# aharmat/mcptam

Measured on AMD Instinct MI355X. Metric: ChainBundle LM iters/sec (4-cam, 200 MKF, 50k pts, 400k meas) @1/2/4/8 GPU, higher is better.
Workload: dtype f64; 1 GPU; metric: 4 cams, 200 MKF, 50000 points, 400000 measurements per rank; parallelism=points sharded x1, poses replicated, allreduce_transport=none

## Files before the change

### include/mcp_ba.h

```cpp
#ifndef MCP_BA_H
#define MCP_BA_H

#include <stddef.h>

#ifdef __cplusplus
extern "C" {
#endif

#define MCP_MAX_CHAIN 8
#define MCP_MAX_INV   31

typedef struct mcp_camera {
  double params[9];
  double image_size[2];
  double affine[4];
  double center[2];
  double min_theta;
  double max_rho;
  double theta_mean;
  double theta_std;
  int    n_inv;
  int    pad_;
  double inv_coeffs[MCP_MAX_INV];
} mcp_camera;
// ... 92 lines not shown
void mcp_ba_struct_cache_stats(long long* hits, long long* misses);
long long mcp_ba_struct_cache_near_hits(void);
void mcp_ba_struct_cache_clear(void);
int mcp_chol_debug_factor(const double* A, int n, const double* b, double* L_out, double* y_out, int* info);
int mcp_chol_time(const double* A, int n, const double* b, int nsys, int reps, int band, double* ms_factor, double* ms_back, double* x);
int mcp_debug_pose_cut(const unsigned char* adjacency, int nf, int max_arcs, int threads, int* order_out, int* segs_out, int* info_out);
int mcp_ba_debug_system(mcp_ba*, double lambda, double* S_rhs_b_out);
int mcp_ba_debug_systems(mcp_ba*, int nsys, const double* lambdas, double* out);
#define MCP_BA_LIN_NONE  0
#define MCP_BA_LIN_QUAD  1
#define MCP_BA_LIN_PIPE  2
#define MCP_BA_LIN_GROUP 3
#define MCP_BA_SCHUR_NONE  0
#define MCP_BA_SCHUR_4     1
#define MCP_BA_SCHUR_GROUP 2
typedef struct mcp_ba_structure {
  int ngroup, grp_pts, nbig, nfl, np;
  int grp_points_max, grp_points_min;
  int grp_poses_max;
  int grp_no_pose;
  int grp_blk_max, grp_inc_max;
  int lin_kernel;
  int lin_generic;
  int schur_kernel;
  int asm_long;
  int max_systems;
} mcp_ba_structure;
int mcp_ba_debug_structure(mcp_ba*, mcp_ba_structure* out);

#define MCP_BA_HEAD_PLAIN 0
#define MCP_BA_HEAD_RANKS 1
#define MCP_BA_HEAD_RIDE  2
#define MCP_BA_HEAD_SMALL 3
#define MCP_BA_HEAD_AHEAD 4
#define MCP_BA_HEAD_LARGE 5
typedef struct mcp_ba_head_report {
  unsigned long long rank;
  double median;
  double sigma[4];
  double robust_chi2;
  double robust_chi2_plain;
// ... 28 lines not shown
```

### mcptam_amd/chain_bundle.py

```python
import ctypes
import os
import time

import numpy as np

from .taylor_camera import camera_array

_HERE = os.path.dirname(os.path.abspath(__file__))
LIB_PATH = os.environ.get("MCP_HIP_LIB") or os.path.join(_HERE, "libmcptam_hip.so")
_LIB = None

c_double_p = ctypes.POINTER(ctypes.c_double)
c_int_p = ctypes.POINTER(ctypes.c_int)
c_ubyte_p = ctypes.POINTER(ctypes.c_ubyte)


class McpBaParams(ctypes.Structure):
    _fields_ = [("max_iterations", ctypes.c_int), ("max_trials_after_failure", ctypes.c_int),
                ("update_percent_limit", ctypes.c_double), ("update_rms_limit", ctypes.c_double),
                ("min_mestimator_sigma", ctypes.c_double), ("disable_convergence", ctypes.c_int),
                ("device", ctypes.c_int), ("profile", ctypes.c_int)]


class McpBaIterLog(ctypes.Structure):
# ... 6 lines not shown
    _fields_ = [("total_ms", ctypes.c_double), ("structure_ms", ctypes.c_double), ("eval_ms", ctypes.c_double),
                ("select_ms", ctypes.c_double), ("linearize_ms", ctypes.c_double), ("schur_ms", ctypes.c_double),
                ("cholesky_ms", ctypes.c_double), ("solve_ms", ctypes.c_double), ("update_ms", ctypes.c_double),
                ("n_linearize", ctypes.c_int), ("n_trials", ctypes.c_int), ("n_solves", ctypes.c_int),
                ("n_spec_hits", ctypes.c_int),
                ("n_collectives_main", ctypes.c_int), ("n_collectives_spec", ctypes.c_int),
                ("collective_bytes_main", ctypes.c_double), ("collective_bytes_spec", ctypes.c_double),
                ("n_median_fast", ctypes.c_int), ("n_persist_fallbacks", ctypes.c_int),
                ("schur_mfma_per_system", ctypes.c_double), ("schur_flops_structural", ctypes.c_double),
                ("chol_flops_plan", ctypes.c_double), ("chol_chains", ctypes.c_int)]


class McpBaStructure(ctypes.Structure):
    _fields_ = [(f, ctypes.c_int) for f in (
        "ngroup", "grp_pts", "nbig", "nfl", "np", "grp_points_max", "grp_points_min", "grp_poses_max", "grp_no_pose",
        "grp_blk_max", "grp_inc_max", "lin_kernel", "lin_generic", "schur_kernel", "asm_long", "max_systems")]


class McpBaHeadReport(ctypes.Structure):
    _fields_ = [("rank", ctypes.c_ulonglong), ("median", ctypes.c_double), ("sigma", ctypes.c_double * 4),
                ("robust_chi2", ctypes.c_double), ("robust_chi2_plain", ctypes.c_double), ("route_sigma", ctypes.c_double * 4),
                ("head_status", ctypes.c_int), ("overflow", ctypes.c_int), ("pred_ok", ctypes.c_int),
                ("select_overflow", ctypes.c_int), ("n_median_fast", ctypes.c_int), ("declined", ctypes.c_int)]


class McpBaTrialReport(ctypes.Structure):
    _fields_ = [(f, ctypes.c_double) for f in ("robust_chi2", "scale_pose", "scale_point", "scale", "ss_pose", "ss_point", "ss")] + \
               [(f, ctypes.c_int) for f in ("ncb", "nbb", "nchain", "npose", "npoint", "nfl", "np", "nmeas", "small_mode", "given_step")]


HEAD_ROUTES = ("plain", "ranks", "ride", "small", "ahead", "large")
LIN_KERNEL_NAMES = ("none", "quad", "pipe", "group")
SCHUR_KERNEL_NAMES = ("none", "schur4", "schur_group")

ALLREDUCE_FN = ctypes.CFUNCTYPE(ctypes.c_int, ctypes.c_void_p, ctypes.c_void_p, ctypes.c_size_t, ctypes.c_void_p)

BA_SYMBOLS = [
    "mcp_last_error", "mcp_device_count", "mcp_ba_create", "mcp_ba_destroy", "mcp_ba_add_pose", "mcp_ba_add_point",
    "mcp_ba_add_meas", "mcp_ba_add_points", "mcp_ba_add_measurements", "mcp_ba_compute", "mcp_ba_converged",
    "mcp_ba_total_iterations", "mcp_ba_get_point", "mcp_ba_get_pose", "mcp_ba_get_points", "mcp_ba_get_poses",
    "mcp_ba_num_outliers", "mcp_ba_get_outliers", "mcp_ba_sigma_squared", "mcp_ba_mean_chi_squared", "mcp_ba_max_cov",
    "mcp_ba_lambda", "mcp_ba_num_iter_logs", "mcp_ba_get_iter_logs", "mcp_ba_get_timing", "mcp_ba_set_allreduce",
    "mcp_ba_prepare", "mcp_ba_eval", "mcp_ba_robust_chi2", "mcp_ba_debug_solve", "mcp_dense_spd_solve",
    "mcp_dense_spd_stress", "mcp_ba_debug_system", "mcp_ba_debug_systems", "mcp_ba_debug_structure", "mcp_ba_debug_head", "mcp_ba_debug_trial", "mcp_chol_debug_factor", "mcp_chol_time", "mcp_debug_pose_cut",
    "mcp_ba_struct_cache_stats", "mcp_ba_struct_cache_near_hits", "mcp_ba_struct_cache_clear",
    "mcp_comm_unique_id", "mcp_comm_init", "mcp_comm_destroy", "mcp_ba_set_comm", "mcp_comm_allreduce", "mcp_comm_allreduce_lane",
]

# ... 274 lines not shown
        out = np.zeros(max(len(lams), 1) * per)
        if self._L.mcp_ba_debug_systems(self._h, len(lams), _dp(lams), _dp(out)) < 0:
            raise RuntimeError("mcp_ba_debug_systems: " + last_error())
        return [(out[q * per:q * per + n * n].reshape(n, n).copy(), out[q * per + n * n:q * per + n * n + n].copy(),
                 out[q * per + n * n + n:(q + 1) * per].copy()) for q in range(len(lams))]

    def DebugStructure(self):
        st = McpBaStructure()
        if self._L.mcp_ba_debug_structure(self._h, ctypes.byref(st)) < 0:
            raise RuntimeError("mcp_ba_debug_structure: " + last_error())
        d = {f: int(getattr(st, f)) for f, _ in McpBaStructure._fields_}
        d["lin_kernel"] = LIN_KERNEL_NAMES[d["lin_kernel"]]
        d["schur_kernel"] = SCHUR_KERNEL_NAMES[d["schur_kernel"]]
        d["lin_generic"] = bool(d["lin_generic"])
        d["asm_long"] = bool(d["asm_long"])
        return d

    def DebugHead(self, route, chi2, prev_median):
        chi2 = np.ascontiguousarray(chi2, dtype=np.float64).reshape(-1)
        rep = McpBaHeadReport()
        if self._L.mcp_ba_debug_head(self._h, HEAD_ROUTES.index(route), _dp(chi2), len(chi2), float(prev_median), ctypes.byref(rep)) < 0:
            raise RuntimeError("mcp_ba_debug_head: " + last_error())
        d = {f: getattr(rep, f) for f, _ in McpBaHeadReport._fields_}
        d["sigma"] = np.array(rep.sigma[:], dtype=np.float64)
        d["route_sigma"] = np.array(rep.route_sigma[:], dtype=np.float64)
        return d

    def DebugTrial(self, lam, x=None):
        rep = McpBaTrialReport()
        nx = self.Prepare()
# ... 128 lines not shown
```

### mcptam_amd/csrc/ba_group.h

```cpp
#pragma once
#include "ba_kernels.h"

namespace mcp {

__device__ inline int tri(int r, int c) { return r*(r + 1)/2 + c; }
constexpr int GRP_TRI = GRP_DOF*(GRP_DOF + 1)/2;

template <int NT>
__device__ inline void flush_group_blocks(const double* Sl, const double* bl, int grp, const DevProblem& P,
                                          double* __restrict__ st_blocks, double* __restrict__ st_rhs) {
  const int b0 = P.g_blk0[grp], nb = P.g_blk0[grp + 1] - b0;
  for (int e = threadIdx.x; e < nb*36; e += NT) {
    const int slot = e/36, w = e - 36*slot;
    const int pr = P.blk_pair[b0 + slot], la = pr >> 4, lb = pr & 15;
    const int r = w/6, c = w - 6*r;
    st_blocks[(size_t)P.blk_dst[b0 + slot]*36 + w] = (la == lb && c > r) ? 0.0 : Sl[tri(6*la + r, 6*lb + c)];
  }
  for (int i = threadIdx.x; i < GRP_DOF; i += NT) {
    const int d = P.rhs_dst[grp*GRP_LMAX + i/6];
    if (d >= 0) st_rhs[(size_t)d*6 + i%6] = bl[i];
  }
}

template <int NT>
// ... 740 lines not shown
    __syncthreads();
    if (t >= GRP_DOF && t < 2*GRP_DOF) rl[t - GRP_DOF] += racc;
    __syncthreads();
    flush_group_blocks<256>(Sl, rl, grp, P, stS, str);
  }
  SCH_LAP(7);
  SCH_OUT();
}
struct AsmPlan {
  int nfp;
  int ntiles;
  const int* tiles;
  const int* pair_id;
  const int* pr_start;
  const int* po_start;
};

#ifndef ASM_NT
#define ASM_NT 1024
#endif
__global__ void __launch_bounds__(ASM_NT)
k_assemble(AsmPlan A, int np, const double* __restrict__ stU, const double* __restrict__ stb,
           const double* __restrict__ stS, const double* __restrict__ str,
           const double* __restrict__ Ubig ,
           double* __restrict__ S, SysBatch sb) {
  const int q = blockIdx.y;
  S += q*sb.sstride; stS += q*sb.ststride; str += q*sb.strstride;
  const double lam = sb.lambda_init[q];
  const int packed = A.tiles[blockIdx.x];
  const int ti = packed >> 16, tj = packed & 0xffff;
  const size_t n2 = (size_t)np*np;
  for (int e = threadIdx.x; e < 1024; e += ASM_NT) {
    const int row = 32*ti + (e >> 5), col = 32*tj + (e & 31);
    if (col >= np || row > np) continue;
    if (row == np) {
      const int a = col/6, r = col - 6*a;
      double b = 0.0, sr = 0.0;
// ... 30 lines not shown
        }
        for (; k + 4 <= k1; k += 4, pu += 144, pw += 144) {
          const double u0 = pu[0], u1 = pu[36], u2 = pu[72], u3 = pu[108];
          const double w0 = pw[0], w1 = pw[36], w2 = pw[72], w3 = pw[108];
          u += u0; u += u1; u += u2; u += u3;
          w += w0; w += w1; w += w2; w += w3;
        }
        for (; k < k1; ++k, pu += 36, pw += 36) { u += pu[0]; w += pw[0]; }
      }
      v = u - w;
      if (Ubig) v += Ubig[(size_t)row*np + col];
      if (row == col) v += lam;
    }
    S[(size_t)row*np + col] = v;
  }
}

constexpr int ASML_LPE = 8;
__device__ inline double asml_tree8(double v) {
  v += wave_xor<1>(v); v += wave_xor<2>(v); v += __shfl_xor(v, 4, 64);
  return v;
}
__device__ inline double asml_part(const double* __restrict__ p, int stride, int n, int l8) {
  const int c0 = (n*l8)/ASML_LPE, c1 = (n*(l8 + 1))/ASML_LPE;
  double a = 0.0;
  int k = c0;
  p += (size_t)c0*stride;
  for (; k + 4 <= c1; k += 4, p += 4*(size_t)stride) {
    const double x0 = p[0], x1 = p[stride], x2 = p[2*(size_t)stride], x3 = p[3*(size_t)stride];
    a += x0; a += x1; a += x2; a += x3;
// ... 80 lines not shown
```

### mcptam_amd/csrc/ba_solver.hip

```cpp
#include <hip/hip_runtime.h>
#include <algorithm>
#include <array>
#include <atomic>
#include <memory>
#include <mutex>
#include <sched.h>
#include <thread>
#include <cfloat>
#include <chrono>
#include <cmath>
#include <cstdio>
#include <cstdlib>
#include <cstring>
#include <condition_variable>
#include <functional>
#include <list>
#include <map>
#include <string>
#include <vector>

#include "../../include/mcp_ba.h"
#include "ba_pool.h"
#include "ba_kernels.h"
#include "ba_select.h"
// ... 282 lines not shown
  P.ok = P.main && P.spec;
  if (getenv("MCP_BA_TRACE")) fprintf(stderr, "[mcp_ba streams] device %d: %d side streams overlap with the main stream%s\n", device, got, calibrate ? "" : " (not measured)");
  return P;
}

struct StructKey {
  unsigned long long h0 = 0, h1 = 0; int npose = 0, npoint = 0, nmeas = 0, nchain = 0, dev = 0, flags = 0;
  bool operator==(const StructKey& o) const { return h0 == o.h0 && h1 == o.h1 && npose == o.npose && npoint == o.npoint && nmeas == o.nmeas && nchain == o.nchain && dev == o.dev && flags == o.flags; }
};
struct StructEntry {
  StructKey key;
  std::vector<int> pose_unk, pt_unk, fp_pose, fl_point, perm;
  std::vector<unsigned char> pose_active, pt_active, pat;
  std::vector<int> chol_segs;
  int nfp = 0, nfl = 0, np = 0, nx = 0, nsp = 0, ninc = 0, nslot = 0, ngroup = 0, nbig = 0, grp_pts = 0, grp_blk_max = 0, grp_inc_max = 0, nrhs_rows = 0;
  size_t nstage = 0; bool asm_long = false, sch4_ok = false, sch4_order = false;
  double m_total = 0, nfl_total = 0, schur_mfma = 0, schur_flops = 0;
  std::vector<size_t> counts;
  StructKey base;
  std::vector<int, NoInitAlloc<int>> add_point, add_chain, add_cam;
  char* dblock = nullptr; size_t dbytes = 0, dcap = 0; int ddev = -1;
  size_t host_bytes() const { return (pose_unk.size() + pt_unk.size() + fp_pose.size() + fl_point.size() + perm.size() + add_point.size() + add_chain.size() + add_cam.size())*4 + pose_active.size() + pt_active.size() + pat.size(); }
  ~StructEntry() { if (dblock) DevCache::get().put(dblock, dcap, ddev); }
};
class StructCache {
 public:
  static StructCache& get() { static StructCache* c = new StructCache(); return *c; }
  bool enabled() const { return budget_ > 0; }
  std::shared_ptr<StructEntry> find(const StructKey& k) {
    std::lock_guard<std::mutex> lk(mu_);
    for (auto it = lru_.begin(); it != lru_.end(); ++it) if ((*it)->key == k) { auto e = *it; lru_.erase(it); lru_.push_front(e); ++hits_; return e; }
// ... 87 lines not shown
    DevBuf<double> xp, xl, p0, p1, p2;
    bool pre_run = false, ahead_enq = false; unsigned long long pre_ticket = 0;
    hipEvent_t ev_tr = nullptr;
    hipEvent_t ev_wf = nullptr;
    hipStream_t st_tr = nullptr;
    hipStream_t tr_stream = nullptr;
    hipEvent_t head_ev = nullptr; bool head_enq = false; int head_state = -1; unsigned long long head_ticket = 0;
    DevBuf<double> trial; DevBuf<SelState> trstate;
    int pred_ok = 0, ovf = 0;
  };
  SpecLane lane[MAX_SYS];
  int spec_trials = 2;
  DevBuf<double> d_ubig;
  DevBuf<double> d_red;
  DevBuf<double> d_stU, d_stb, d_stS, d_str, d_udiag;
  DevBuf<int> d_g_blk0, d_asm_tiles, d_pair_id, d_pr_start, d_blk_dst, d_po_start, d_rhs_dst;
  DevBuf<unsigned char> d_blk_pair;
  int grp_blk_max = 0;
  int head_ahead_for = -1;
  bool head_ahead_want = false; int dbg_head_ahead = 0;
  int head_ahead(int w);
  int large_head_ahead = 0;
  struct HeadScratch { unsigned int* hist = nullptr; double* vals = nullptr; double* part = nullptr; double* out = nullptr; double* rs = nullptr; };
  HeadScratch hsc[2*MAX_SYS]; DevBuf<double> d_headbuf;
  hipStream_t st_h = nullptr; bool st_h_own = false;
  unsigned long long head_ticket_ctr = 0;
  int head_par = 0, acc_head_q = -1, dbg_head_miss = 0;
  const double* start_blk = nullptr;
  unsigned int* head_hist(int q) { return hsc[head_par*MAX_SYS + q].hist; }
  int enqueue_head(hipStream_t s, int q, int w, bool side);
  int wait_head(int q);
// ... 17 lines not shown
  int grp_lmax_pol = env_on("MCP_BA_GROUP_LMAX13", true) ? S4_LMAX : GRP_LMAX;
  bool sch4_on = env_on("MCP_BA_SCHUR4", true), sch4_ok = false;
  double schur_mfma = 0, schur_flops = 0;
  std::vector<unsigned char> last_pat;
  std::string launch_err;
  void note_launch(const char* k) { const hipError_t e = hipGetLastError(); if (e != hipSuccess && e != hipErrorNotReady && launch_err.empty()) launch_err = std::string(k) + ": " + hipGetErrorString(e); }
  std::shared_ptr<StructEntry> pending_entry;
  StructKey cache_key, cache_base; bool cache_insert = false;
  int n_masked = 0; int near_miss_on = 1;
  unsigned long long med_rank() const { return (unsigned long long)n_masked + (unsigned long long)(m_total/2); }
  DevBuf<int> d_m_last;
  bool lin_pipe = env_on("MCP_BA_LIN_PIPE", true);
  DevBuf<int> d_g_order, d_sp_unk;
  bool sch4_order = false;
  bool asm_long = false;
  int grp_inc_max = 0;
  size_t nstage = 0;
  int nrhs_rows = 0;
  AsmPlan A;
  DevBuf<double> d_V, d_g, d_W, d_Vinv, d_xl, d_xp_good, d_xl_good, d_err;
  DevBuf<double> d_selvals;
  DevBuf<double> d_seltab;
  int sel_cap = 4096;
  DevBuf<double> d_xp_cand;
  DevBuf<double> d_part0, d_part1, d_part2, d_res, d_sigma, d_hist, d_cov;
  static constexpr int MAX_DIAG_PARTS = 256;
  static int max_diag_parts(int np_, int nfl_) { return std::min(MAX_DIAG_PARTS, (std::max(np_, nfl_) + 1023)/1024); }
  DevBuf<unsigned char> d_headl; bool headl_clean = false; int head_large_on = 0; int hl_grid = 0;
  bool use_head_large() const { return head_large_on && robust && !multi() && !small_mode() && P.nmeas > 0 && hl_grid > 0 && d_headl.p != nullptr; }
  int head_large(int w, int off, double* sig_copy2);
// ... 1359 lines not shown
  B.hold_arena(st);
  HostStruct& H = B.H;
#define CP(x) H.x.assign(x.begin(), x.end())
  CP(m_pt); CP(m_chain); CP(m_sp); CP(slot_start); CP(slot_unk); CP(slot_inc); CP(l_i0); CP(l_i1); CP(l_sp); CP(inc_unk); CP(sp_pt); CP(sp_m); CP(sp_i);
  CP(g_sp0); CP(g_pose); CP(g_blk0); CP(pair_id); CP(pr_start); CP(blk_dst); CP(po_start); CP(rhs_dst); CP(m_cam); CP(slot_first); CP(sp_big); CP(slot_lp);
  CP(inc_lp); CP(inc_mixed); CP(blk_pair); CP(m_mask); CP(m_u); CP(m_v); CP(m_om);
#undef CP
  return finish_prepare(B);
}

struct mcp_ba::BlockLayout {
  struct Item { const void* src; size_t bytes, off; bool direct; };
  std::vector<Item> items; std::vector<size_t> counts;
  size_t total = 0, staged = 0; char* base = nullptr;
  static size_t al(size_t x) { return (x + 255) & ~(size_t)255; }
  std::vector<int> chain_len, chain_pose, pose_unk, pt_chain, pt_unk, sp_unk, g_order; std::vector<unsigned char> pt_fixed;
  std::vector<int, NoInitAlloc<int>> m_last;
};

int mcp_ba::finish_prepare(StructBuild& B) {
  pending_entry.reset();
  const int nmeas = B.hit ? B.hit->key.nmeas : B.nmeas;
  const int nblk = (std::max(nmeas, nfl) + 255)/256 + 1;
  BlockLayout L;
  launch_choices(B);
  if (layout_block(B, L)) return -1;
  if (B.hit ? upload_hit_numbers(B, L) : upload_cold(L)) return -1;
  B.lap("  upload enqueued");
  if (!B.hit && cache_insert && make_cache_entry(B, L)) return -1;
  read_call_knobs();
  if (alloc_work_buffers(nmeas, nblk) || head_scratch(nmeas, nblk) || poison_test_aid() || pinned_mailbox(nblk) || zero_fill() || fill_param_blocks(nmeas)) return -1;
  B.lap("alloc+upload");
  return publish(B);
}

void mcp_ba::launch_choices(StructBuild& B) {
  const StructEntry* hit = B.hit.get(); const HostStruct& H = B.H;
  sch4_ok = ngroup > 0;
  if (hit) sch4_ok = hit->sch4_ok;
  else for (int gi = 0; gi < ngroup && sch4_ok; ++gi) if (H.g_pose[(size_t)gi*GRP_LMAX + S4_LMAX] >= 0) sch4_ok = false;
  schur_mfma = schur_flops = 0;
  if (hit) { schur_mfma = hit->schur_mfma; schur_flops = hit->schur_flops; }
  else if ((prm.profile || cache_insert) && ngroup) schur_work(B);
  if (hit) asm_long = hit->asm_long;
  else {
    const size_t npairs = H.pr_start.empty() ? 0 : H.pr_start.size() - 1;
    asm_long = npairs > 0 && nstage >= 48*npairs;
    if (const char* e = getenv("MCP_BA_ASM_LONG")) asm_long = atoi(e) != 0 && npairs > 0;
  }
}

void mcp_ba::schur_work(StructBuild& B) {
  const HostStruct& H = B.H;
  const int T = finish_threads(B.nmeas);
  std::vector<double> pm(T, 0.0), pf(T, 0.0);
  auto body = [&](int tid) {
    double sm = 0, sf = 0;
    for (int gi = (int)((long)ngroup*tid/T), ge = (int)((long)ngroup*(tid + 1)/T); gi < ge; ++gi) {
      int npl = 0; for (int k = 0; k < GRP_LMAX; ++k) if (H.g_pose[(size_t)gi*GRP_LMAX + k] >= 0) npl = k + 1;
      const int ntile = (6*npl + 15)/16;
      for (int s0 = H.g_sp0[gi]; s0 < H.g_sp0[gi + 1]; s0 += 16) {
        unsigned tm = 0;
        for (int sp = s0; sp < std::min(s0 + 16, H.g_sp0[gi + 1]); ++sp) {
          if (H.sp_big[sp]) continue;
// ... 19 lines not shown
  for (int i = 0; i < npoint; ++i) { L.pt_chain[i] = points[i].chain; L.pt_unk[i] = points[i].unk; L.pt_fixed[i] = (unsigned char)points[i].fixed; }
  L.sp_unk.resize(hit ? 0 : nsp);
  if (!hit) for (int sp = 0; sp < nsp; ++sp) L.sp_unk[sp] = H.sp_big[sp] ? -1 : L.pt_unk[H.sp_pt[sp]];
  sch4_order = hit ? hit->sch4_order : (sch4_on && sch4_ok && ngroup > 512 && env_on("MCP_BA_SCHUR4_ORDER", true));
  if (sch4_order && !hit) {
    std::vector<int> cost(ngroup);
    for (int gi = 0; gi < ngroup; ++gi) {
      int npl = 0; for (int k = 0; k < GRP_LMAX; ++k) if (H.g_pose[(size_t)gi*GRP_LMAX + k] >= 0) npl = k + 1;
      const int nt = (6*npl + 15)/16;
      cost[gi] = nt*(nt + 1)/2*((H.g_sp0[gi + 1] - H.g_sp0[gi] + 15)/16);
    }
    L.g_order.resize(ngroup);
    for (int gi = 0; gi < ngroup; ++gi) L.g_order[gi] = gi;
    std::stable_sort(L.g_order.begin(), L.g_order.end(), [&](int a, int b) { return cost[a] > cost[b]; });
  }
  L.m_last.resize(hit ? 0 : nmeas);
  if (!hit) {
    auto& m_last = L.m_last; const int T = finish_threads(nmeas);
    run_ranges(T, [&](int tid) { for (long j = (long)nmeas*tid/T, e = (long)nmeas*(tid + 1)/T; j < e; ++j) { const int oc = H.m_chain[j]; m_last[j] = oc*MAXC + chains[oc].len - 1; } });
  }
}

int mcp_ba::layout_block(StructBuild& B, BlockLayout& L) {
  const StructEntry* hit = B.hit.get(); const HostStruct& H = B.H;
  small_arrays(B, L);
  L.items.reserve(48); L.counts.reserve(48);
  size_t& total = L.total; auto al = BlockLayout::al;
  size_t nadd = 0;
  auto add = [&](auto& dbuf, const auto& vec, bool pinned) {
    using E = typename std::remove_reference<decltype(vec)>::type::value_type;
// ... 8 lines not shown
    if (!direct) L.staged += al(std::max<size_t>(bytes, 1));
    total += al(std::max<size_t>(bytes, 1));
  };
  add(d_cams, cams, false); add(d_chain_len, L.chain_len, false); add(d_chain_pose, L.chain_pose, false); add(d_pose_unk, L.pose_unk, false);
  add(d_pt_chain, L.pt_chain, false); add(d_pt_unk, L.pt_unk, false); add(d_pt_fixed, L.pt_fixed, false);
  add(d_m_pt, H.m_pt, true); add(d_m_chain, H.m_chain, true); add(d_m_cam, H.m_cam, true); add(d_m_mask, H.m_mask, true);
  add(d_m_u, H.m_u, true); add(d_m_v, H.m_v, true); add(d_m_omega, H.m_om, true); add(d_slot_start, H.slot_start, true);
  add(d_slot_unk, H.slot_unk, true); add(d_slot_inc, H.slot_inc, true); add(d_l_i0, H.l_i0, true); add(d_l_i1, H.l_i1, true);
  add(d_inc_unk, H.inc_unk, true); add(d_fl_point, fl_point, false); add(d_sp_pt, H.sp_pt, true); add(d_sp_m, H.sp_m, true);
  add(d_sp_i, H.sp_i, true); add(d_sp_big, H.sp_big, true); add(d_m_sp, H.m_sp, true); add(d_l_sp, H.l_sp, true);
  add(d_g_sp0, H.g_sp0, true); add(d_g_pose, H.g_pose, true); add(d_slot_lp, H.slot_lp, true); add(d_slot_first, H.slot_first, true);
  add(d_inc_lp, H.inc_lp, true); add(d_inc_mixed, H.inc_mixed, true); add(d_g_blk0, H.g_blk0, true); add(d_blk_pair, H.blk_pair, true);
  add(d_asm_tiles, plan.all_tiles, false); add(d_pair_id, H.pair_id, true); add(d_pr_start, H.pr_start, true); add(d_blk_dst, H.blk_dst, true);
  add(d_po_start, H.po_start, true); add(d_rhs_dst, H.rhs_dst, true);
  add(d_sp_unk, L.sp_unk, false); add(d_g_order, L.g_order, false); add(d_m_last, L.m_last, false);
  if (d_struct.alloc(total)) return -1;
  char* const base = L.base = d_struct.p;
  auto fix = [&](auto& dbuf) { dbuf.p = reinterpret_cast<decltype(dbuf.p)>(base + reinterpret_cast<size_t>(dbuf.p)); };
  fix(d_cams); fix(d_chain_len); fix(d_chain_pose); fix(d_pose_unk); fix(d_pt_chain); fix(d_pt_unk); fix(d_pt_fixed);
  fix(d_m_pt); fix(d_m_chain); fix(d_m_cam); fix(d_m_mask); fix(d_m_u); fix(d_m_v); fix(d_m_omega); fix(d_slot_start);
  fix(d_slot_unk); fix(d_slot_inc); fix(d_l_i0); fix(d_l_i1); fix(d_inc_unk); fix(d_fl_point); fix(d_sp_pt); fix(d_sp_m);
  fix(d_sp_i); fix(d_sp_big); fix(d_m_sp); fix(d_l_sp); fix(d_g_sp0); fix(d_g_pose); fix(d_slot_lp); fix(d_slot_first);
  fix(d_inc_lp); fix(d_inc_mixed); fix(d_g_blk0); fix(d_blk_pair); fix(d_asm_tiles); fix(d_pair_id); fix(d_pr_start); fix(d_blk_dst);
  fix(d_po_start); fix(d_rhs_dst); fix(d_sp_unk); fix(d_g_order); fix(d_m_last);
  return 0;
}

int mcp_ba::upload_hit_numbers(StructBuild& B, BlockLayout& L) {
  const StructEntry* hit = B.hit.get(); const int nmeas = hit->key.nmeas;
  if (hit->dbytes != L.total) { set_err("structure cache: layout mismatch"); return -1; }
  HIPCK(hipMemcpyAsync(L.base, hit->dblock, L.total, hipMemcpyDeviceToDevice, st));
  const size_t nm = (size_t)nmeas;
  double* vals = (double*)pinned_arena().alloc((3*nm + 1)*sizeof(double));
  {
    const int T = finish_threads(nmeas);
    const int* pm = perm.data(); const HMeas* ms = meas.data();
    run_ranges(T, [&](int tid) {
      for (size_t j = nm*tid/T, e = nm*(tid + 1)/T; j < e; ++j) {
        if (pm[j] < 0) { vals[j] = 0.0; vals[nm + j] = 0.0; vals[2*nm + j] = 0.0; continue; }
// ... 44 lines not shown
  {
    e->add_point.resize(nmeas); e->add_chain.resize(nmeas); e->add_cam.resize(nmeas);
    const int T = finish_threads(nmeas);
    run_ranges(T, [&](int tid) {
      const long j0 = (long)nmeas*tid/T, j1 = (long)nmeas*(tid + 1)/T;
      if (j1 > j0) { std::memcpy(e->add_point.data() + j0, meas_point.data() + j0, (size_t)(j1 - j0)*sizeof(int)); std::memcpy(e->add_chain.data() + j0, meas_chain.data() + j0, (size_t)(j1 - j0)*sizeof(int)); }
      for (long j = j0; j < j1; ++j) e->add_cam[j] = meas[j].cam;
    });
  }
  e->pose_unk.resize(npose); e->pose_active.resize(npose); e->pt_unk.resize(npoint); e->pt_active.resize(npoint);
  for (int i = 0; i < npose; ++i) { e->pose_unk[i] = poses[i].unk; e->pose_active[i] = (unsigned char)poses[i].active; }
  for (int i = 0; i < npoint; ++i) { e->pt_unk[i] = points[i].unk; e->pt_active[i] = (unsigned char)points[i].active; }
  e->fp_pose = fp_pose; e->fl_point = fl_point; e->perm = perm; e->pat = last_pat; e->chol_segs = chol_segs;
  e->nfp = nfp; e->nfl = nfl; e->np = np; e->nx = nx; e->nsp = nsp; e->ninc = ninc; e->nslot = nslot; e->ngroup = ngroup; e->nbig = nbig;
  e->grp_pts = grp_pts; e->grp_blk_max = grp_blk_max; e->grp_inc_max = grp_inc_max; e->nrhs_rows = nrhs_rows; e->nstage = nstage;
  e->asm_long = asm_long; e->sch4_ok = sch4_ok; e->sch4_order = sch4_order; e->m_total = m_total; e->nfl_total = nfl_total;
  e->schur_mfma = schur_mfma; e->schur_flops = schur_flops; e->counts = L.counts;
  e->dblock = (char*)DevCache::get().take(std::max<size_t>(total, 1), &e->dcap, &e->ddev);
  if (e->dblock) {
    e->dbytes = total;
    HIPCK(hipMemcpyAsync(e->dblock, L.base, total, hipMemcpyDeviceToDevice, st));
    pending_entry = e;
  }
  B.lap("  cache entry");
  return 0;
}

void mcp_ba::read_call_knobs() {
  { const char* e = getenv("MCP_BA_SPECULATE"); if (e) speculate = atoi(e); }
  { const char* e = getenv("MCP_BA_SPECULATE_ADAPT"); if (e) spec_adapt = atoi(e); }
  { const char* e = getenv("MCP_BA_LIN_JOIN"); if (e) lin_join_full = atoi(e); }
// ... 100 lines not shown
}

int mcp_ba::fill_param_blocks(int nmeas) {
  const int npose = (int)poses.size(), npoint = (int)points.size(); const size_t nc = chains.size();
  P.cams = d_cams.p; P.ncam = (int)cams.size(); P.nchain = (int)nc; P.chain_len = d_chain_len.p; P.chain_pose = d_chain_pose.p;
  P.npose = npose; P.pose_unk = d_pose_unk.p; P.npoint = npoint; P.pt_chain = d_pt_chain.p; P.pt_unk = d_pt_unk.p;
  P.pt_fixed = d_pt_fixed.p; P.nmeas = nmeas; P.m_pt = d_m_pt.p; P.m_chain = d_m_chain.p; P.m_cam = d_m_cam.p;
  P.m_mask = d_m_mask.p; P.m_u = d_m_u.p; P.m_v = d_m_v.p; P.m_omega = d_m_omega.p; P.slot_start = d_slot_start.p;
  P.slot_unk = d_slot_unk.p; P.slot_inc = d_slot_inc.p; P.nfl = nfl; P.ninc = ninc; P.np = np;
  P.l_i0 = d_l_i0.p; P.l_i1 = d_l_i1.p; P.inc_unk = d_inc_unk.p; P.fl_point = d_fl_point.p; P.robust = robust;
  P.nsp = nsp; P.ngroup = ngroup; P.sp_pt = d_sp_pt.p; P.sp_m = d_sp_m.p; P.sp_i = d_sp_i.p; P.sp_big = d_sp_big.p;
  P.m_sp = d_m_sp.p; P.l_sp = d_l_sp.p; P.g_sp0 = d_g_sp0.p; P.g_pose = d_g_pose.p; P.slot_lp = d_slot_lp.p;
  P.slot_first = d_slot_first.p; P.inc_lp = d_inc_lp.p; P.inc_mixed = d_inc_mixed.p;
  P.g_blk0 = d_g_blk0.p; P.blk_pair = d_blk_pair.p; P.blk_dst = d_blk_dst.p; P.rhs_dst = d_rhs_dst.p; P.sp_unk = d_sp_unk.p; P.m_last = d_m_last.p;
  A.nfp = nfp; A.ntiles = (int)plan.all_tiles.size(); A.tiles = d_asm_tiles.p; A.pair_id = d_pair_id.p;
  A.pr_start = d_pr_start.p; A.po_start = d_po_start.p;
  {
    static std::atomic<unsigned long long> sch_attr{0};
    const unsigned long long bit = 1ull << (device & 63);
    if (!(sch_attr.load(std::memory_order_relaxed) & bit)) {
      HIPCK(hipFuncSetAttribute((const void*)k_schur_group, hipFuncAttributeMaxDynamicSharedMemorySize, (int)SCH_LDS_BYTES));
      sch_attr.fetch_or(bit, std::memory_order_relaxed);
    }
  }
  return 0;
}

int mcp_ba::publish(StructBuild& B) {
  if (upload_state()) { pending_entry.reset(); return -1; }
  {
    const hipError_t es = hipStreamSynchronize(st);
// ... 321 lines not shown
  sbfull.sstride = sb.sstride; sbfull.vstride = sb.vstride; sbfull.ststride = sb.ststride; sbfull.strstride = sb.strstride;
  double* Sq = d_red.p + q0*red_stride; double* Vq = d_Vinv.p + q0*vinv_stride;
  double* stSq = d_stS.p + q0*sb.ststride; double* strq = d_str.p + q0*sb.strstride; int* failq = d_fail.p + q0;
  if (main_stream) tic(ST_SCHUR);
  const int sk = schur_kernel();
  if (sk == MCP_BA_SCHUR_4)
    hipLaunchKernelGGL(k_schur4, dim3(ngroup), dim3(256), S4_LDS_BYTES, s, P, nsys, (const int*)(sch4_order ? d_g_order.p : nullptr), (const double*)d_V.p, (const double*)d_g.p, (const double*)d_W.p, Vq, stSq, strq, failq, sb);
  else if (sk == MCP_BA_SCHUR_GROUP) hipLaunchKernelGGL(k_schur_group, dim3(ngroup, nsys), dim3(256), SCH_LDS_BYTES, s, P, sb.lambda[0], d_V.p, d_g.p, d_W.p, Vq, stSq, strq, failq, sb);
  if (nfl && ngroup) note_launch("k_schur4 / k_schur_group");
  else if (ngroup && nstage) {
    HIPCK(hipMemsetAsync(stSq, 0, (size_t)nsys*nstage*36*sizeof(double), s));
    HIPCK(hipMemsetAsync(strq, 0, (size_t)nsys*nrhs_rows*6*sizeof(double), s));
  }
  if (np && asm_long) hipLaunchKernelGGL(k_assemble_long, dim3(A.ntiles*32, nsys), dim3(32*ASML_LPE), 0, s, A, np, (const double*)d_stU.p, (const double*)d_stb.p,
                             (const double*)stSq, (const double*)strq, (const double*)Ubig(), Sq, sb);
  else if (np) hipLaunchKernelGGL(k_assemble, dim3(A.ntiles, nsys), dim3(ASM_NT), 0, s, A, np, (const double*)d_stU.p, (const double*)d_stb.p,
                             (const double*)stSq, (const double*)strq, (const double*)Ubig(), Sq, sb);
  if (nfl && nbig) hipLaunchKernelGGL(k_schur, dim3(1, nsys), dim3(256), 0, s, P, sb.lambda[0], d_V.p, d_g.p, d_W.p, Vq, Sq, Sq + (size_t)np*np, failq, sb);
  if (main_stream) toc();
#ifdef MCP_SCH_PROF
  {
    HIPCK(hipStreamSynchronize(s));
    unsigned long long pr[64]; hipMemcpyFromSymbol(pr, HIP_SYMBOL(g_sch_prof), sizeof pr);
    double a[8] = {0}; int cnt = 0;
    for (int b2 = 0; b2 < 8; ++b2) { const unsigned long long* q = pr + 8*b2; if (!q[0]) continue; for (int i2 = 0; i2 < 8; ++i2) a[i2] += (double)q[i2]; ++cnt; }
    if (cnt && sch4_on && sch4_ok)
      fprintf(stderr, "[sch4 prof] prologue %.0f  clear+scatter %.0f  barrier %.0f  prefetch+mfma %.0f  barrier %.0f  flush %.0f  (cycles of wavefront 0, %d systems, %d groups)\n",
              a[0]/cnt, a[1]/cnt, a[2]/cnt, a[3]/cnt, a[4]/cnt, a[5]/cnt, nsys, cnt);
    else if (cnt) fprintf(stderr, "[sch prof] prologue %.0f  inverse+barrier %.0f  scatter %.0f  prefetch+barrier %.0f  mfma %.0f  rhs %.0f  barrier+clear %.0f  flush %.0f  (cycles, %d systems, %d groups)\n",
                     a[0]/cnt, a[1]/cnt, a[2]/cnt, a[3]/cnt, a[4]/cnt, a[5]/cnt, a[6]/cnt, a[7]/cnt, nsys, cnt);
  }
// ... 975 lines not shown
    std::vector<int> sp0((size_t)h->ngroup + 1), gp((size_t)h->ngroup*GRP_LMAX);
    HIPCK(hipStreamSynchronize(h->st));
    HIPCK(hipMemcpy(sp0.data(), h->d_g_sp0.p, sp0.size()*sizeof(int), hipMemcpyDeviceToHost));
    HIPCK(hipMemcpy(gp.data(), h->d_g_pose.p, gp.size()*sizeof(int), hipMemcpyDeviceToHost));
    r.grp_points_min = sp0[1] - sp0[0];
    for (int gi = 0; gi < h->ngroup; ++gi) {
      const int npt = sp0[gi + 1] - sp0[gi];
      int npl = 0; for (int k = 0; k < GRP_LMAX; ++k) if (gp[(size_t)gi*GRP_LMAX + k] >= 0) npl = k + 1;
      r.grp_points_max = std::max(r.grp_points_max, npt); r.grp_points_min = std::min(r.grp_points_min, npt);
      r.grp_poses_max = std::max(r.grp_poses_max, npl);
      if (!npl) ++r.grp_no_pose;
    }
  }
  r.lin_kernel = h->lin_kernel(); r.lin_generic = h->lin_generic() ? 1 : 0; r.schur_kernel = h->schur_kernel();
  r.asm_long = (h->np && h->asm_long) ? 1 : 0; r.max_systems = h->batch_capacity();
  *out = r;
  return 0;
}

int mcp_ba_debug_head(mcp_ba* h, int route, const double* chi2, int n, double prev_median, mcp_ba_head_report* out) {
  static const char* const names[6] = { "plain", "ranks", "ride", "small", "ahead", "large" };
  if (!chi2 || !out) { set_err("mcp_ba_debug_head: no chi2 array or no report block"); return -1; }
  if (route < 0 || route > 5) { set_err("mcp_ba_debug_head: unknown route (MCP_BA_HEAD_PLAIN .. MCP_BA_HEAD_LARGE)"); return -1; }
  if (h->dirty && h->prepare()) return -1;
  HIPCK(hipSetDevice(h->device));
  char msg[256];
  if (n != h->P.nmeas) { snprintf(msg, sizeof msg, "mcp_ba_debug_head: chi2 holds %d values, the handle has %d measurements", n, h->P.nmeas); set_err(msg); return -1; }
  const char* why = nullptr;
  if (!h->robust) why = "the handle has no robust kernel";
  else if (h->P.nmeas == 0 || h->m_total == 0) why = "the map has no measurement";
// ... 453 lines not shown
```

Measured before the change: 2097 LM iterations/s (x map shards).

## Add pose-pair task-table assembly kernel for reduced camera system

Adds a new default assembly path that builds a host-side task table with one task per 6x6 pose-pair block, sorted by walk length, plus zero-fill and RHS tasks. Each 64-lane group covers one system and one block, walking the staged U and S contributions. This replaces the per-tile 1024-thread assembly kernel. The aim is to balance load and cut idle threads when the map is sparse. The cost is a larger task table and more blocks, and it is only used when the long-assembly and big-point paths are off.

Result: faster. 2186 LM iterations/s (x map shards) (median of 6 runs) (+4.2%).

```diff
diff --git a/include/mcp_ba.h b/include/mcp_ba.h
--- a/include/mcp_ba.h
+++ b/include/mcp_ba.h
@@ -130,6 +130,10 @@
 #define MCP_BA_SCHUR_NONE  0
 #define MCP_BA_SCHUR_4     1
 #define MCP_BA_SCHUR_GROUP 2
+#define MCP_BA_ASM_NONE  0
+#define MCP_BA_ASM_PAIR  1
+#define MCP_BA_ASM_TILES 2
+#define MCP_BA_ASM_LONG  3
 typedef struct mcp_ba_structure {
   int ngroup, grp_pts, nbig, nfl, np;
   int grp_points_max, grp_points_min;
@@ -141,6 +145,7 @@
   int schur_kernel;
   int asm_long;
   int max_systems;
+  int asm_kernel;
 } mcp_ba_structure;
 int mcp_ba_debug_structure(mcp_ba*, mcp_ba_structure* out);
 
diff --git a/mcptam_amd/chain_bundle.py b/mcptam_amd/chain_bundle.py
--- a/mcptam_amd/chain_bundle.py
+++ b/mcptam_amd/chain_bundle.py
@@ -44,7 +44,7 @@
 class McpBaStructure(ctypes.Structure):
     _fields_ = [(f, ctypes.c_int) for f in (
         "ngroup", "grp_pts", "nbig", "nfl", "np", "grp_points_max", "grp_points_min", "grp_poses_max", "grp_no_pose",
-        "grp_blk_max", "grp_inc_max", "lin_kernel", "lin_generic", "schur_kernel", "asm_long", "max_systems")]
+        "grp_blk_max", "grp_inc_max", "lin_kernel", "lin_generic", "schur_kernel", "asm_long", "max_systems", "asm_kernel")]
 
 
 class McpBaHeadReport(ctypes.Structure):
@@ -62,6 +62,7 @@
 HEAD_ROUTES = ("plain", "ranks", "ride", "small", "ahead", "large")
 LIN_KERNEL_NAMES = ("none", "quad", "pipe", "group")
 SCHUR_KERNEL_NAMES = ("none", "schur4", "schur_group")
+ASM_KERNEL_NAMES = ("none", "pair", "tiles", "long")
 
 ALLREDUCE_FN = ctypes.CFUNCTYPE(ctypes.c_int, ctypes.c_void_p, ctypes.c_void_p, ctypes.c_size_t, ctypes.c_void_p)
 
@@ -366,6 +367,7 @@
         d["schur_kernel"] = SCHUR_KERNEL_NAMES[d["schur_kernel"]]
         d["lin_generic"] = bool(d["lin_generic"])
         d["asm_long"] = bool(d["asm_long"])
+        d["asm_kernel"] = ASM_KERNEL_NAMES[d["asm_kernel"]]
         return d
 
     def DebugHead(self, route, chi2, prev_median):
diff --git a/mcptam_amd/csrc/ba_group.h b/mcptam_amd/csrc/ba_group.h
--- a/mcptam_amd/csrc/ba_group.h
+++ b/mcptam_amd/csrc/ba_group.h
@@ -778,13 +778,21 @@
   const int* pair_id;
   const int* pr_start;
   const int* po_start;
+  int ntasks, nwalk;
+  const int4* tasks;
 };
+
+constexpr int ASMP_ZB = 8;
+constexpr int ASMP_POSE_BITS = 11;
+constexpr int ASMP_RHS = 1 << (2*ASMP_POSE_BITS + 4);
+constexpr int ASMP_RHS_POSES = 10;
+__host__ __device__ inline int asmp_task(int a, int b, int mask) { return a | (b << ASMP_POSE_BITS) | (mask << 2*ASMP_POSE_BITS); }
 
 #ifndef ASM_NT
 #define ASM_NT 1024
 #endif
 __global__ void __launch_bounds__(ASM_NT)
-k_assemble(AsmPlan A, int np, const double* __restrict__ stU, const double* __restrict__ stb,
+k_assemble_tiles(AsmPlan A, int np, const double* __restrict__ stU, const double* __restrict__ stb,
            const double* __restrict__ stS, const double* __restrict__ str,
            const double* __restrict__ Ubig ,
            double* __restrict__ S, SysBatch sb) {
@@ -845,6 +853,72 @@
     }
     S[(size_t)row*np + col] = v;
   }
+}
+
+template <int STRIDE>
+__device__ inline void asm_walk2(const double* __restrict__ pu, const double* __restrict__ pw, int n, double& u, double& w) {
+  int k = 0;
+  for (; k + 16 <= n; k += 16, pu += 16*STRIDE, pw += 16*STRIDE) {
+    double uu[16], ww[16];
+#pragma unroll
+    for (int j = 0; j < 16; ++j) { uu[j] = pu[STRIDE*j]; ww[j] = pw[STRIDE*j]; }
+#pragma unroll
+    for (int j = 0; j < 16; ++j) { u += uu[j]; w += ww[j]; }
+  }
+  for (; k + 4 <= n; k += 4, pu += 4*STRIDE, pw += 4*STRIDE) {
+    const double u0 = pu[0], u1 = pu[STRIDE], u2 = pu[2*STRIDE], u3 = pu[3*STRIDE];
+    const double w0 = pw[0], w1 = pw[STRIDE], w2 = pw[2*STRIDE], w3 = pw[3*STRIDE];
+    u += u0; u += u1; u += u2; u += u3;
+    w += w0; w += w1; w += w2; w += w3;
+  }
+  for (; k < n; ++k, pu += STRIDE, pw += STRIDE) { u += pu[0]; w += pw[0]; }
+}
+__device__ inline void asmp_store(int word, int lane, int np, double u, double w, double lam, double* __restrict__ S) {
+  const int a = word & ((1 << ASMP_POSE_BITS) - 1), b = (word >> ASMP_POSE_BITS) & ((1 << ASMP_POSE_BITS) - 1), mask = (word >> 2*ASMP_POSE_BITS) & 15;
+  const int r = lane/6, c = lane - 6*r, row = 6*a + r, col = 6*b + c;
+  const int quad = 2*((row >> 5) != ((6*a) >> 5)) + ((col >> 5) != ((6*b) >> 5));
+  if (!((mask >> quad) & 1)) return;
+  double v = 0.0;
+  if (col <= row) {
+    v = u - w;
+    if (row == col) v += lam;
+  }
+  S[(size_t)row*np + col] = v;
+}
+__global__ void __launch_bounds__(64*MAX_SYS)
+k_assemble(AsmPlan A, int np, const double* __restrict__ stU, const double* __restrict__ stb,
+           const double* __restrict__ stS, const double* __restrict__ str, double* __restrict__ S, SysBatch sb) {
+  const int q = (int)threadIdx.x >> 6, lane = threadIdx.x & 63;
+  S += q*sb.sstride; stS += q*sb.ststride; str += q*sb.strstride;
+  const double lam = sb.lambda_init[q];
+  if ((int)blockIdx.x >= A.nwalk) {
+    if (lane >= 36) return;
+    const int t0 = A.nwalk + ((int)blockIdx.x - A.nwalk)*ASMP_ZB;
+    int word[ASMP_ZB];
+#pragma unroll
+    for (int i = 0; i < ASMP_ZB; ++i) word[i] = t0 + i < A.ntasks ? A.tasks[t0 + i].x : -1;
+#pragma unroll
+    for (int i = 0; i < ASMP_ZB; ++i) if (word[i] >= 0) asmp_store(word[i], lane, np, 0.0, 0.0, lam, S);
+    return;
+  }
+  const int4 task = A.tasks[blockIdx.x];
+  if (task.x & ASMP_RHS) {
+    const int a = (task.x & ((1 << ASMP_POSE_BITS) - 1)) + lane/6, r = lane%6;
+    if (lane >= 6*ASMP_RHS_POSES || a >= A.nfp) return;
+    const int k0 = A.po_start[a], n = A.po_start[a + 1] - k0;
+    double b = 0.0, sr = 0.0;
+    asm_walk2<6>(stb + (size_t)k0*6 + r, str + (size_t)k0*6 + r, n, b, sr);
+    const int col = 6*a + r;
+    const size_t n2 = (size_t)np*np;
+    S[n2 + col] = b - sr;
+    S[n2 + np + col] = b;
+    return;
+  }
+  if (lane >= 36) return;
+  double u = 0.0, w = 0.0;
+  const int a = task.x & ((1 << ASMP_POSE_BITS) - 1), b = (task.x >> ASMP_POSE_BITS) & ((1 << ASMP_POSE_BITS) - 1);
+  if (a != b || lane%6 <= lane/6) asm_walk2<36>(stU + (size_t)task.y*36 + lane, stS + (size_t)task.y*36 + lane, task.z, u, w);
+  asmp_store(task.x, lane, np, u, w, lam, S);
 }
 
 constexpr int ASML_LPE = 8;
diff --git a/mcptam_amd/csrc/ba_solver.hip b/mcptam_amd/csrc/ba_solver.hip
--- a/mcptam_amd/csrc/ba_solver.hip
+++ b/mcptam_amd/csrc/ba_solver.hip
@@ -320,7 +320,7 @@
   std::vector<unsigned char> pose_active, pt_active, pat;
   std::vector<int> chol_segs;
   int nfp = 0, nfl = 0, np = 0, nx = 0, nsp = 0, ninc = 0, nslot = 0, ngroup = 0, nbig = 0, grp_pts = 0, grp_blk_max = 0, grp_inc_max = 0, nrhs_rows = 0;
-  size_t nstage = 0; bool asm_long = false, sch4_ok = false, sch4_order = false;
+  size_t nstage = 0; bool asm_long = false, sch4_ok = false, sch4_order = false; int n_asm_walk = 0;
   double m_total = 0, nfl_total = 0, schur_mfma = 0, schur_flops = 0;
   std::vector<size_t> counts;
   StructKey base;
@@ -438,7 +438,7 @@
   DevBuf<double> d_ubig;
   DevBuf<double> d_red;
   DevBuf<double> d_stU, d_stb, d_stS, d_str, d_udiag;
-  DevBuf<int> d_g_blk0, d_asm_tiles, d_pair_id, d_pr_start, d_blk_dst, d_po_start, d_rhs_dst;
+  DevBuf<int> d_g_blk0, d_asm_tiles, d_pair_id, d_pr_start, d_blk_dst, d_po_start, d_rhs_dst, d_asm_tasks;
   DevBuf<unsigned char> d_blk_pair;
   int grp_blk_max = 0;
   int head_ahead_for = -1;
@@ -486,6 +486,8 @@
   DevBuf<int> d_g_order, d_sp_unk;
   bool sch4_order = false;
   bool asm_long = false;
+  bool asm_pair = false;
+  int n_asm_tasks = 0, n_asm_walk = 0;
   int grp_inc_max = 0;
   size_t nstage = 0;
   int nrhs_rows = 0;
@@ -1875,7 +1877,7 @@
   std::vector<Item> items; std::vector<size_t> counts;
   size_t total = 0, staged = 0; char* base = nullptr;
   static size_t al(size_t x) { return (x + 255) & ~(size_t)255; }
-  std::vector<int> chain_len, chain_pose, pose_unk, pt_chain, pt_unk, sp_unk, g_order; std::vector<unsigned char> pt_fixed;
+  std::vector<int> chain_len, chain_pose, pose_unk, pt_chain, pt_unk, sp_unk, g_order, asm_tasks; std::vector<unsigned char> pt_fixed;
   std::vector<int, NoInitAlloc<int>> m_last;
 };
 
@@ -1903,12 +1905,55 @@
   schur_mfma = schur_flops = 0;
   if (hit) { schur_mfma = hit->schur_mfma; schur_flops = hit->schur_flops; }
   else if ((prm.profile || cache_insert) && ngroup) schur_work(B);
+  n_asm_walk = hit ? hit->n_asm_walk : 0;
   if (hit) asm_long = hit->asm_long;
   else {
     const size_t npairs = H.pr_start.empty() ? 0 : H.pr_start.size() - 1;
     asm_long = npairs > 0 && nstage >= 48*npairs;
     if (const char* e = getenv("MCP_BA_ASM_LONG")) asm_long = atoi(e) != 0 && npairs > 0;
   }
+  asm_pair = np > 0 && !asm_long && !nbig && env_on("MCP_BA_ASM_PAIR", true);
+}
+
+static int asm_task_table(int nfp, int np, const int* pair_id, const int* pr_start, const int* po_start, const std::vector<int>& tiles, std::vector<int>& tasks) {
+  tasks.clear();
+  if (nfp <= 0 || nfp >= (1 << ASMP_POSE_BITS)) return 0;
+  const int ntc = (np + CH_NB - 1)/CH_NB, ntr = np/CH_NB + 1;
+  static_assert(CH_NB == 32, "k_assemble's quadrant test shifts by 5");
+  std::vector<unsigned char> in_plan((size_t)ntr*ntc, 0);
+  for (int t : tiles) in_plan[(size_t)(t >> 16)*ntc + (t & 0xffff)] = 1;
+  auto tile = [&](int ti, int tj) { return ti >= tj && in_plan[(size_t)ti*ntc + tj]; };
+  std::vector<int> word, first, len;
+  for (int a = 0; a < nfp; ++a) {
+    const int ti0 = (6*a)/CH_NB, ti1 = (6*a + 5)/CH_NB;
+    for (int b = 0; b < nfp; ++b) {
+      const int tj0 = (6*b)/CH_NB, tj1 = (6*b + 5)/CH_NB;
+      int mask = tile(ti0, tj0) ? 1 : 0;
+      if (tj1 != tj0 && tile(ti0, tj1)) mask |= 2;
+      if (ti1 != ti0 && tile(ti1, tj0)) mask |= 4;
+      if (ti1 != ti0 && tj1 != tj0 && tile(ti1, tj1)) mask |= 8;
+      if (!mask) continue;
+      const int pid = a >= b ? pair_id[(size_t)a*nfp + b] : -1;
+      word.push_back(asmp_task(a, b, mask)); first.push_back(pid >= 0 ? pr_start[pid] : 0); len.push_back(pid >= 0 ? pr_start[pid + 1] - pr_start[pid] : 0);
+    }
+  }
+  for (int a = 0; a < nfp; a += ASMP_RHS_POSES) {
+    int n = 0;
+    for (int p = a; p < std::min(a + ASMP_RHS_POSES, nfp); ++p) n = std::max(n, po_start[p + 1] - po_start[p]);
+    word.push_back(asmp_task(a, 0, 0) | ASMP_RHS); first.push_back(0); len.push_back(std::max(n, 1));
+  }
+  int lmax = 0; for (int n : len) lmax = std::max(lmax, n);
+  std::vector<int> pos(lmax + 2, 0);
+  for (int n : len) pos[lmax - n + 1]++;
+  for (int i = 0; i <= lmax; ++i) pos[i + 1] += pos[i];
+  tasks.resize(4*word.size());
+  int nwalk = 0;
+  for (size_t i = 0; i < word.size(); ++i) {
+    int* t = &tasks[4*(size_t)pos[lmax - len[i]]++];
+    t[0] = word[i]; t[1] = first[i]; t[2] = (word[i] & ASMP_RHS) ? 0 : len[i]; t[3] = 0;
+    if (len[i] > 0) ++nwalk;
+  }
+  return nwalk;
 }
 
 void mcp_ba::schur_work(StructBuild& B) {
@@ -1958,6 +2003,7 @@
     for (int gi = 0; gi < ngroup; ++gi) L.g_order[gi] = gi;
     std::stable_sort(L.g_order.begin(), L.g_order.end(), [&](int a, int b) { return cost[a] > cost[b]; });
   }
+  if (!hit && np > 0 && !asm_long && !nbig) n_asm_walk = asm_task_table(nfp, np, H.pair_id.data(), H.pr_start.data(), H.po_start.data(), plan.all_tiles, L.asm_tasks);
   L.m_last.resize(hit ? 0 : nmeas);
   if (!hit) {
     auto& m_last = L.m_last; const int T = finish_threads(nmeas);
@@ -1996,6 +2042,8 @@
   add(d_asm_tiles, plan.all_tiles, false); add(d_pair_id, H.pair_id, true); add(d_pr_start, H.pr_start, true); add(d_blk_dst, H.blk_dst, true);
   add(d_po_start, H.po_start, true); add(d_rhs_dst, H.rhs_dst, true);
   add(d_sp_unk, L.sp_unk, false); add(d_g_order, L.g_order, false); add(d_m_last, L.m_last, false);
+  add(d_asm_tasks, L.asm_tasks, false); n_asm_tasks = (int)(L.counts.back()/4);
+  asm_pair = asm_pair && n_asm_tasks > 0;
   if (d_struct.alloc(total)) return -1;
   char* const base = L.base = d_struct.p;
   auto fix = [&](auto& dbuf) { dbuf.p = reinterpret_cast<decltype(dbuf.p)>(base + reinterpret_cast<size_t>(dbuf.p)); };
@@ -2004,7 +2052,7 @@
   fix(d_slot_unk); fix(d_slot_inc); fix(d_l_i0); fix(d_l_i1); fix(d_inc_unk); fix(d_fl_point); fix(d_sp_pt); fix(d_sp_m);
   fix(d_sp_i); fix(d_sp_big); fix(d_m_sp); fix(d_l_sp); fix(d_g_sp0); fix(d_g_pose); fix(d_slot_lp); fix(d_slot_first);
   fix(d_inc_lp); fix(d_inc_mixed); fix(d_g_blk0); fix(d_blk_pair); fix(d_asm_tiles); fix(d_pair_id); fix(d_pr_start); fix(d_blk_dst);
-  fix(d_po_start); fix(d_rhs_dst); fix(d_sp_unk); fix(d_g_order); fix(d_m_last);
+  fix(d_po_start); fix(d_rhs_dst); fix(d_sp_unk); fix(d_g_order); fix(d_m_last); fix(d_asm_tasks);
   return 0;
 }
 
@@ -2079,7 +2127,7 @@
   e->fp_pose = fp_pose; e->fl_point = fl_point; e->perm = perm; e->pat = last_pat; e->chol_segs = chol_segs;
   e->nfp = nfp; e->nfl = nfl; e->np = np; e->nx = nx; e->nsp = nsp; e->ninc = ninc; e->nslot = nslot; e->ngroup = ngroup; e->nbig = nbig;
   e->grp_pts = grp_pts; e->grp_blk_max = grp_blk_max; e->grp_inc_max = grp_inc_max; e->nrhs_rows = nrhs_rows; e->nstage = nstage;
-  e->asm_long = asm_long; e->sch4_ok = sch4_ok; e->sch4_order = sch4_order; e->m_total = m_total; e->nfl_total = nfl_total;
+  e->asm_long = asm_long; e->n_asm_walk = n_asm_walk; e->sch4_ok = sch4_ok; e->sch4_order = sch4_order; e->m_total = m_total; e->nfl_total = nfl_total;
   e->schur_mfma = schur_mfma; e->schur_flops = schur_flops; e->counts = L.counts;
   e->dblock = (char*)DevCache::get().take(std::max<size_t>(total, 1), &e->dcap, &e->ddev);
   if (e->dblock) {
@@ -2210,7 +2258,7 @@
   P.slot_first = d_slot_first.p; P.inc_lp = d_inc_lp.p; P.inc_mixed = d_inc_mixed.p;
   P.g_blk0 = d_g_blk0.p; P.blk_pair = d_blk_pair.p; P.blk_dst = d_blk_dst.p; P.rhs_dst = d_rhs_dst.p; P.sp_unk = d_sp_unk.p; P.m_last = d_m_last.p;
   A.nfp = nfp; A.ntiles = (int)plan.all_tiles.size(); A.tiles = d_asm_tiles.p; A.pair_id = d_pair_id.p;
-  A.pr_start = d_pr_start.p; A.po_start = d_po_start.p;
+  A.pr_start = d_pr_start.p; A.po_start = d_po_start.p; A.ntasks = n_asm_tasks; A.nwalk = n_asm_walk; A.tasks = (const int4*)d_asm_tasks.p;
   {
     static std::atomic<unsigned long long> sch_attr{0};
     const unsigned long long bit = 1ull << (device & 63);
@@ -2562,7 +2610,9 @@
   }
   if (np && asm_long) hipLaunchKernelGGL(k_assemble_long, dim3(A.ntiles*32, nsys), dim3(32*ASML_LPE), 0, s, A, np, (const double*)d_stU.p, (const double*)d_stb.p,
                              (const double*)stSq, (const double*)strq, (const double*)Ubig(), Sq, sb);
-  else if (np) hipLaunchKernelGGL(k_assemble, dim3(A.ntiles, nsys), dim3(ASM_NT), 0, s, A, np, (const double*)d_stU.p, (const double*)d_stb.p,
+  else if (np && asm_pair) hipLaunchKernelGGL(k_assemble, dim3(A.nwalk + (A.ntasks - A.nwalk + ASMP_ZB - 1)/ASMP_ZB), dim3(64*nsys), 0, s, A, np, (const double*)d_stU.p, (const double*)d_stb.p,
+                             (const double*)stSq, (const double*)strq, Sq, sb);
+  else if (np) hipLaunchKernelGGL(k_assemble_tiles, dim3(A.ntiles, nsys), dim3(ASM_NT), 0, s, A, np, (const double*)d_stU.p, (const double*)d_stb.p,
                              (const double*)stSq, (const double*)strq, (const double*)Ubig(), Sq, sb);
   if (nfl && nbig) hipLaunchKernelGGL(k_schur, dim3(1, nsys), dim3(256), 0, s, P, sb.lambda[0], d_V.p, d_g.p, d_W.p, Vq, Sq, Sq + (size_t)np*np, failq, sb);
   if (main_stream) toc();
@@ -3568,6 +3618,7 @@
   }
   r.lin_kernel = h->lin_kernel(); r.lin_generic = h->lin_generic() ? 1 : 0; r.schur_kernel = h->schur_kernel();
   r.asm_long = (h->np && h->asm_long) ? 1 : 0; r.max_systems = h->batch_capacity();
+  r.asm_kernel = !h->np ? MCP_BA_ASM_NONE : h->asm_long ? MCP_BA_ASM_LONG : h->asm_pair ? MCP_BA_ASM_PAIR : MCP_BA_ASM_TILES;
   *out = r;
   return 0;
 }
```
